# primus-labs/primus-fhe

Hardware: AMD Instinct MI355X
Metric: NTT/sec at N=2^16, 3-prime RNS (forward limb-NTTs, batch 4096 RNS polynomials per GPU) (higher is better)
Workload: dtype u64; 1 GPU; BASELINE configs[2] shape: N=2^16, 3-prime RNS (61-bit), batch=4096 per GPU, forward DCRT NTT in place (config 3'); log_n=16, batch_per_gpu=4096

## Files before the change

primus-fhe_amd/csrc/pfhe_ntt.hip:

```cpp
#include <algorithm>
#include <cstdio>
#include <cstdlib>
#include <vector>

#include "pfhe_common.hpp"
#include "pfhe_modmath.hpp"
#include "pfhe_ntt_device.hpp"

namespace pfhe {

template <bool INV>
__global__ void ntt_tiny_kernel(u64 *__restrict__ data, const NttPrime *__restrict__ primes, u32 L, u32 log_n,
                                u64 npolys, u32 lazy) {
    u64 pid = (u64)blockIdx.x * blockDim.x + threadIdx.x;
    if (pid >= npolys) return;
    const ShoupArith ar(primes + pid % L);
    const u32 n = 1u << log_n;
    u64 *x = data + pid * n;
    if (!INV) {
        for (u32 p = log_n; p-- > 0;) {
            for (u32 e = 0; e < n; ++e) {
                if (e & (1u << p)) continue;
                fwd_bfly(ar, x[e], x[e | (1u << p)], ar.fwd_tw((n + e) >> (p + 1)));
            }
// ... 72 lines not shown
}
template <class A, int K, int VEC, bool INV, bool FINAL>
__global__ __launch_bounds__(256) void ntt_strided_oop_kernel(u64 *__restrict__ dst, const u64 *__restrict__ src,
                                                              const NttPrime *__restrict__ primes, u32 L, u32 log_n, u32 log_s,
                                                              u64 total_threads, u32 lazy) {
    strided_pass_body<A, K, VEC, INV, FINAL, false>(dst, src, primes, L, log_n, log_s,
                                                    (u64)blockIdx.x * blockDim.x + threadIdx.x, total_threads, lazy);
}


struct NoHook {
    __device__ __forceinline__ void operator()() const {}
};
template <class A, int LOGB, bool INV, bool MUL, int LOGE = 4, class Hook = NoHook, bool NTIO = false, class Hook2 = NoHook>
__device__ __forceinline__ void block_pass_body(u64 *__restrict__ data, const u64 *src, const NttPrime *__restrict__ primes, u32 L,
                                                u32 log_n, u64 total_blocks, u32 lazy, const u64 *__restrict__ mul,
                                                u64 mul_polys, u64 *__restrict__ lds_raw, u64 first_block,
                                                Hook after_stage = Hook(), Hook2 before_store = Hook2()) {
    using Cfg = BlockCfg<LOGB, LOGE>;
    constexpr bool kNt = !std::is_same<Hook, NoHook>::value || NTIO;
    constexpr int NV = Cfg::E / 2;
    constexpr bool kWL = wave_local_vectors<LOGB, LOGE>() && !(INV && A::kMont && !std::is_same<Hook, NoHook>::value);
    const u32 tid = threadIdx.x;
    const u32 sub = Cfg::BPW == 1 ? 0u : tid / Cfg::TPB;
    const u32 lt = Cfg::BPW == 1 ? tid : tid % Cfg::TPB;
    u64 blk = first_block * Cfg::BPW + sub;
    const bool valid = blk < total_blocks;
    if (!valid) blk = 0;
    const u32 log_nb = log_n - LOGB;
    const u64 pid = blk >> log_nb;
    const u32 bi = (u32)(blk & ((1ull << log_nb) - 1));
    const u32 limb = (u32)(pid % L);
    const A ar(primes + limb);
    const u32 n = 1u << log_n;
    const u32 eblk = bi << LOGB;
    u64 *__restrict__ gptr = data + pid * n + eblk;
    const u64 *sgptr = src + pid * n + eblk;
    u64 *__restrict__ lds = lds_raw + (size_t)sub * Cfg::LDS_WORDS;

    constexpr bool kDirectLoad = !INV && !MUL && Cfg::BPW == 1 && (LOGB - LOGE) >= 6 &&
                                 !std::is_same<Hook, NoHook>::value && !A::kPacked
        ;
    u64x2 io[NV];
    u64 x[Cfg::E];
    if constexpr (kDirectLoad) {
#pragma unroll
        for (int k = 0; k < Cfg::E; ++k)
#ifdef PFHE_NOMEM
            x[k] = (u64)lt * 0x9E3779B97F4A7C15ull + (u64)k + lazy;
#else
            x[k] = valid ? __builtin_nontemporal_load(sgptr + ((u32)k << (LOGB - LOGE)) + lt) : 0ull;
#endif
        after_stage();
        block_forward_core<A, LOGB, false, LOGE>(ar, x, lds, n, eblk, lt, lazy != 0);
        lds_put_layout<0, LOGE>(x, lds, lt);
        sync_vectors_layout0<LOGB, LOGE, kWL>();
        lds_get_vectors<LOGB, LOGE, kWL>(io, lds, lt);
        before_store();
#ifdef PFHE_NOMEM
        if (lazy == 0xdeadu)
#endif
        if (valid) store_block_vectors<LOGB, LOGE, kNt, kWL>(io, gptr, lt);
        return;
    }
    if (valid) {
        load_block_vectors<LOGB, LOGE, kNt, kWL>(io, sgptr, lt);
    } else {
#pragma unroll
        for (int j = 0; j < NV; ++j) io[j] = u64x2{0, 0};
    }
    if constexpr (MUL) {
        u64x2 mv[NV];
        if (valid) {
            const u64 mpoly = mul_polys == (u64)L ? (u64)limb : pid;
            load_block_vectors<LOGB, LOGE, kNt, kWL>(mv, mul + mpoly * n + eblk, lt);
        } else {
#pragma unroll
            for (int j = 0; j < NV; ++j) mv[j] = u64x2{0, 0};
        }
#pragma unroll
        for (int j = 0; j < NV; ++j) {
            io[j].x = ar.mul_any(io[j].x, mv[j].x);
            io[j].y = ar.mul_any(io[j].y, mv[j].y);
        }
    }
    lds_put_vectors<LOGB, LOGE, kWL>(io, lds, lt);
    if constexpr (INV) sync_vectors_layout0<LOGB, LOGE, kWL>();
    else __syncthreads();
    if constexpr (!INV) after_stage();
    if constexpr (!INV) {
        lds_get_layout<LOGB - LOGE, LOGE>(x, lds, lt);
        block_forward_core<A, LOGB, false, LOGE>(ar, x, lds, n, eblk, lt, lazy != 0);
        lds_put_layout<0, LOGE>(x, lds, lt);
    } else {
        lds_get_layout<0, LOGE>(x, lds, lt);
        block_inverse_core<A, LOGB, false, LOGE, Hook>(ar, x, lds, n, eblk, lt, log_n == LOGB, lazy != 0, after_stage);
        constexpr bool kDirectStore = Cfg::BPW == 1 && (LOGB - LOGE) >= 6 && !A::kPacked
            ;
        if constexpr (kDirectStore) {
            before_store();
            if (valid) {
#pragma unroll
                for (int k = 0; k < Cfg::E; ++k)
                    gstore<(kNt && (std::is_same<Hook, NoHook>::value || kPipeIntermediateNt))>(
                        gptr + ((u32)k << (LOGB - LOGE)) + lt, x[k]);
            }
            return;
// ... 144 lines not shown

template <class A, int LOGB, bool INV, bool MUL>
__device__ __forceinline__ void ntt_pipe_body(
    u64 *__restrict__ blk_data, u64 blk_total, u64 *__restrict__ str_data, u64 str_total,
    const NttPrime *__restrict__ primes, u32 L, u32 lazy, const u64 *__restrict__ mul, u64 mul_polys) {
    constexpr int K = 4, TPB = BlockCfg<LOGB>::TPB;
    static_assert(BlockCfg<LOGB>::BPW == 1 && (1 << LOGB) / TPB == (1 << K), "16 blocks and 16 chunks per polynomial");
    constexpr u32 log_n = LOGB + K, n = 1u << log_n;
    extern __shared__ __attribute__((aligned(16))) u64 lds_raw[];
    const u64 chunk = blockIdx.x;
    const bool has_str = chunk < str_total;
    u64 *__restrict__ sp = str_data + (chunk >> 4) * n + (chunk & 15) * TPB + threadIdx.x;
    u64 sx[1 << K][1];
    const auto issue = [&]() {
        if (has_str) {
#pragma unroll
#ifdef PFHE_NOMEM
            for (int k = 0; k < (1 << K); ++k) sx[k][0] = (u64)threadIdx.x * 0xBF58476D1CE4E5B9ull + (u64)k + lazy;
#else
            for (int k = 0; k < (1 << K); ++k) sx[k][0] = __builtin_nontemporal_load(sp + ((u64)k << LOGB));
#endif
        }
    };
    const auto landed = [&]() {
        if (!INV && has_str) {
#pragma unroll
            for (int k = 0; k < (1 << K); ++k) asm volatile("" : "+v"(sx[k][0]));
        }
    };
    if (chunk < blk_total) {
        block_pass_body<A, LOGB, INV, MUL, 4, decltype(issue), false, decltype(landed)>(
            blk_data, blk_data, primes, L, log_n, blk_total, INV ? 0u : lazy, mul, mul_polys, lds_raw, chunk, issue, landed);
    } else {
        issue();
        landed();
    }
    if (has_str) {
        const A ar(primes + (chunk >> 4) % L);
        if constexpr (!INV) strided_forward_regs<A, K, 1, true>(ar, sx, n, 0u, LOGB);
        else strided_inverse_regs<A, K, 1, true>(ar, sx, n, 0u, LOGB, lazy != 0);
#ifdef PFHE_NOMEM
        if (lazy == 0xdeadu)
#endif
#pragma unroll
        for (int k = 0; k < (1 << K); ++k) gstore<(INV || kPipeIntermediateNt)>(sp + ((u64)k << LOGB), sx[k][0]);
    }
}

template <class A, int LOGB>
__global__ __launch_bounds__(BlockCfg<LOGB>::THREADS) __attribute__((amdgpu_waves_per_eu(4, 4))) void ntt_pipe_fwd_kernel(
    u64 *__restrict__ blk_data, u64 blk_total, u64 *__restrict__ str_data, u64 str_total,
    const NttPrime *__restrict__ primes, u32 L, u32 lazy) {
    ntt_pipe_body<A, LOGB, false, false>(blk_data, blk_total, str_data, str_total, primes, L, lazy, nullptr, 0);
}
template <class A, int LOGB, bool MUL>
__global__ __launch_bounds__(BlockCfg<LOGB>::THREADS) __attribute__((amdgpu_waves_per_eu(4, 4))) void ntt_pipe_inv_kernel(
    u64 *__restrict__ blk_data, u64 blk_total, u64 *__restrict__ str_data, u64 str_total,
    const NttPrime *__restrict__ primes, u32 L, u32 lazy, const u64 *__restrict__ mul, u64 mul_polys) {
    ntt_pipe_body<A, LOGB, true, MUL>(blk_data, blk_total, str_data, str_total, primes, L, lazy, mul, mul_polys);
}

template <class A, int LOGB, class HookA = NoHook, class HookM = NoHook, class HookL = NoLateHook, bool NT = false, bool MNT = false>
__device__ __forceinline__ void block_mid_body(const A &ar, u64 *__restrict__ gptr, const u64 *__restrict__ mptr, bool valid,
                                               u32 n, u32 eblk, bool final_block, u64 *__restrict__ lds,
                                               HookA after_load = HookA(), HookM mid = HookM(), HookL late = HookL()) {
    using Cfg = BlockCfg<LOGB>;
    static_assert(Cfg::BPW == 1 && LOGB - 4 >= 6, "one block per workgroup, whole waves per register layout");
    constexpr int NV = Cfg::E / 2, POS0 = LOGB - 4;
    u64 x[Cfg::E];
    {
        const u32 lt = opaque_tid();
#pragma unroll
        for (int k = 0; k < Cfg::E; ++k) x[k] = valid ? __builtin_nontemporal_load(gptr + ((u32)k << POS0) + lt) : 0ull;
        after_load();
        block_forward_core<A, LOGB, false, 4, NoLateHook, true>(ar, x, lds, n, eblk, lt, true);
        lds_put_layout<0>(x, lds, lt);
    }
    {
        const u32 lt = opaque_tid();
        u64x2 io[NV], mv[NV];
        if (valid) {
            load_block_vectors<LOGB, 4, MNT>(mv, mptr, lt);
        } else {
#pragma unroll
            for (int j = 0; j < NV; ++j) mv[j] = u64x2{0, 0};
        }
        sync_vectors_layout0<LOGB>();
        lds_get_vectors<LOGB>(io, lds, lt);
#pragma unroll
        for (int j = 0; j < NV; ++j) {
            io[j].x = ar.mul_any(io[j].x, mv[j].x);
            io[j].y = ar.mul_any(io[j].y, mv[j].y);
        }
        lds_put_vectors<LOGB>(io, lds, lt);
    }
    mid();
    sync_vectors_layout0<LOGB>();
    {
        const u32 lt = opaque_tid();
        lds_get_layout<0>(x, lds, lt);
        block_inverse_core<A, LOGB, false, 4, HookL>(ar, x, lds, n, eblk, lt, final_block, false, late);
    }
    if (valid) {
        const u32 lt = opaque_tid();
#pragma unroll
        for (int k = 0; k < Cfg::E; ++k) gstore<NT>(gptr + ((u32)k << POS0) + lt, x[k]);
// ... 306 lines not shown
        }
        return dispatch_strided<A, false, false>(k, data, primes, L, log_n, log_s, npolys, false, s);
    }
    if (i == 0) return dispatch_strided<A, true, true>(k, data, primes, L, log_n, log_s, npolys, lazy, s);
    return dispatch_strided<A, true, false>(k, data, primes, L, log_n, log_s, npolys, false, s);
}

int pass_dev(const NttPlan &plan, bool persistent, const NttPrime *primes, u32 L, u32 log_n, int arith, u64 *data, u64 npolys,
             bool inverse, int index, bool lazy, hipStream_t s, const u64 *mul, u64 mul_polys) {
    if (index < 0 || index >= plan.passes()) return PFHE_ERR_BAD_ARGUMENT;
    if (plan.tiny) {
        if (arith == kArithB32 || mul) return PFHE_ERR_UNSUPPORTED;
        return launch_tiny(inverse, primes, L, log_n, data, npolys, lazy, s);
    }
    if (persistent)
        return with_arith(arith, [&](auto a) {
            using A = typename decltype(a)::type;
            return inverse ? launch_persist<A, true>(data, primes, L, npolys, lazy, s)
                           : launch_persist<A, false>(data, primes, L, npolys, lazy, s);
        });
    return with_arith<true>(arith, [&](auto a) {
        return run_pass<typename decltype(a)::type>(plan, primes, L, log_n, data, npolys, inverse, index, lazy, s, mul, mul_polys);
    });
}

void pass_name(const NttPlan &plan, bool inverse, int index, char *buf, size_t cap) {
    if (plan.tiny) {
        std::snprintf(buf, cap, "ntt_tiny_kernel");
        return;
    }
    const int block_at = inverse ? 0 : plan.n_strided;
    if (index == block_at) {
        std::snprintf(buf, cap, "ntt_block_kernel<%d,%s>", plan.block_log, inverse ? "inv" : "fwd");
    } else {
        const int i = inverse ? plan.n_strided - index : index;
        std::snprintf(buf, cap, "ntt_strided_kernel<K=%d,%s>", plan.strided[i], inverse ? "inv" : "fwd");
    }
}

}

static int env_int(const char *name, int lo, int hi) {
    const char *e = std::getenv(name);
    if (!e) return 0;
    const int v = std::atoi(e);
    return v >= lo && v <= hi ? v : 0;
}

NttTuning NttTuning::from_env() {
    NttTuning t;
    t.pipe_tiles = env_int("PFHE_PIPE_TILES", 2, 4096);
    t.pipelined = std::getenv("PFHE_DISABLE_PIPELINED") == nullptr;
    t.pipelined_min_mb = env_int("PFHE_PIPELINED_MIN_MB", 1, 1 << 20);
    return t;
}

NttPlan make_ntt_plan(u32 log_n, int arith) {
    NttPlan p;
    if (log_n <= 3) {
        p.tiny = true;
        return p;
    }
    if (log_n <= kMaxSinglePassLog) {
        p.block_log = (int)log_n;
        return p;
    }
    p.block_log = kTwoPassBlockLog;
    if (arith == kArithB32 && log_n == 15) p.block_log = 11;
    int rest = (int)log_n - p.block_log;
    int passes = (rest + 4) / 5;
    for (int i = 0; i < passes; ++i) {
        int k = (rest + (passes - i) - 1) / (passes - i);
        p.strided[p.n_strided++] = k;
        rest -= k;
    }
    return p;
}

int ntt_num_passes(u32 log_n, int arith) { return make_ntt_plan(log_n, arith).passes(); }

void ntt_pass_name(u32 log_n, bool inverse, int index, char *buf, size_t cap, int arith) {
    pass_name(make_ntt_plan(log_n, arith), inverse, index, buf, cap);
}

int ntt_pass_dev(const NttPrime *primes, u32 L, u32 log_n, int arith, u64 *data, u64 npolys, bool inverse, int index,
                 bool lazy, hipStream_t s, const u64 *mul, u64 mul_polys) {
    const NttPlan plan = make_ntt_plan(log_n, arith);
    return pass_dev(plan, mul == nullptr && takes_persistent(plan, arith, npolys), primes, L, log_n, arith, data, npolys,
                    inverse, index, lazy, s, mul, mul_polys);
}

namespace {
constexpr u64 kPipelinedMinBytes = 256ull << 20;
constexpr u64 kPipelinedTileBytes = 256ull << 20;
constexpr int kPipelinedMaxTiles = 64;

int pipelined_tiles(const NttPlan &plan, u32 L, u32 log_n, int arith, u64 npolys, bool inverse, bool has_mul,
                    const NttTuning &tune) {
    const u64 bytes = (npolys << log_n) * sizeof(u64);
    const bool b32 = arith == kArithB32;
    const bool shape = log_n == (b32 ? 15u : 16u) && plan.n_strided == 1 && plan.block_log == (b32 ? 11 : 12);
    if (!(tune.pipelined && shape && (!has_mul || inverse) && npolys % L == 0 &&
          bytes >= (tune.pipelined_min_mb ? (u64)tune.pipelined_min_mb << 20
                                           : b32 ? 4 * kPipelinedMinBytes : kPipelinedMinBytes)))
        return 0;
    const u64 tile_bytes = b32 ? 2 * kPipelinedTileBytes : kPipelinedTileBytes;
    int pt = tune.pipe_tiles ? tune.pipe_tiles
                                : (int)std::min<u64>((bytes + tile_bytes / 2) / tile_bytes, (u64)kPipelinedMaxTiles);
    if (pt < 2) pt = 2;
    if (pt > kPipelinedMaxTiles) pt = kPipelinedMaxTiles;
    if ((u64)pt > npolys / L) pt = (int)(npolys / L);
    return pt;
}

enum class NttOp { kTransform, kInverseMul, kPolymul };
struct NttForm {
    enum Kind { kPasses, kPersistent, kPipelined } kind = kPasses;
    int tiles = 0;
};
NttForm ntt_form(const NttPlan &plan, u32 L, u32 log_n, int arith, u64 npolys, bool inverse, NttOp op, const NttTuning &tune) {
    NttForm f;
    f.tiles = pipelined_tiles(plan, L, log_n, arith, npolys, inverse, op != NttOp::kTransform, tune);
    if (f.tiles >= 1) f.kind = NttForm::kPipelined;
    else if (op != NttOp::kInverseMul && takes_persistent(plan, arith, npolys)) f.kind = NttForm::kPersistent;
    return f;
}

struct PipeTiles {
    u64 *data;
    u64 npolys;
    const u64 *mul;
    u64 mul_polys;
    u32 L, log_n;
    int block_log, tiles;
    struct Tile {
        u64 *ptr = nullptr;
        u64 blocks = 0;
        const u64 *mul = nullptr;
        u64 mul_polys = 0;
    };
    Tile operator[](int k) const {
        Tile t;
        if (k < 0 || k >= tiles) return t;
        const u64 units = npolys / L, u0 = units * (u64)k / (u64)tiles, u1 = units * (u64)(k + 1) / (u64)tiles;
        t.ptr = data + ((u0 * L) << log_n);
        t.blocks = ((u1 - u0) * L) << (log_n - (u32)block_log);
        if (mul) {
            const bool each = mul_polys == npolys;
            t.mul = each ? mul + ((u0 * L) << log_n) : mul;
            t.mul_polys = each ? (u1 - u0) * L : mul_polys;
        }
        return t;
    }
};
}

template <class A, int LOGB>
static int transform_pipelined(const NttPrime *primes, u32 L, u64 *data, u64 npolys, bool inverse, bool lazy,
                               hipStream_t s, int tiles, const u64 *mul, u64 mul_polys) {
    constexpr size_t lds_bytes = (size_t)BlockCfg<LOGB>::LDS_WORDS * sizeof(u64);
    constexpr u32 threads = BlockCfg<LOGB>::THREADS;
    const PipeTiles split{data, npolys, mul, mul_polys, L, LOGB + 4, LOGB, tiles};
    for (int k = 0; k <= tiles; ++k) {
        const PipeTiles::Tile b = split[inverse ? k : k - 1], st = split[inverse ? k - 1 : k];
        const u64 grid = std::max(b.blocks, st.blocks);
        if constexpr (!A::kPacked) {
            if (inverse && mul) {
                PFHE_TRY((launch<ntt_pipe_inv_kernel<A, LOGB, true>>(grid, threads, lds_bytes, s, b.ptr, b.blocks, st.ptr, st.blocks,
                                                                     primes, L, lazy ? 1u : 0u, b.mul, b.mul_polys)));
                continue;
            }
        }
        if (inverse)
            PFHE_TRY((launch<ntt_pipe_inv_kernel<A, LOGB, false>>(grid, threads, lds_bytes, s, b.ptr, b.blocks, st.ptr, st.blocks,
                                                                  primes, L, lazy ? 1u : 0u, b.mul, b.mul_polys)));
        else
            PFHE_TRY((launch<ntt_pipe_fwd_kernel<A, LOGB>>(grid, threads, lds_bytes, s, b.ptr, b.blocks, st.ptr, st.blocks, primes,
                                                           L, lazy ? 1u : 0u)));
    }
    return PFHE_OK;
}

int ntt_transform_form(u32 L, u32 log_n, int arith, u64 npolys, bool inverse, const NttTuning &tune, char *buf, size_t cap) {
    const NttPlan plan = make_ntt_plan(log_n, arith);
    const NttForm form = ntt_form(plan, L, log_n, arith, npolys, inverse, NttOp::kTransform, tune);
    if (form.kind == NttForm::kPipelined) {
        std::snprintf(buf, cap, inverse ? "ntt_pipe_inv_kernel" : "ntt_pipe_fwd_kernel");
        return form.tiles + 1;
    }
    if (form.kind == NttForm::kPersistent) {
        std::snprintf(buf, cap, "ntt_persist_kernel<14,%s>", inverse ? "inv" : "fwd");
        return 1;
    }
    size_t at = 0;
    buf[0] = 0;
    for (int i = 0; i < plan.passes() && at + 1 < cap; ++i) {
        char one[96];
        pass_name(plan, inverse, i, one, sizeof one);
        at += (size_t)std::snprintf(buf + at, cap - at, "%s%s", i ? " + " : "", one);
    }
    return plan.passes();
}

static int transform(const NttPrime *primes, u32 L, u32 log_n, int arith, u64 *data, u64 npolys, bool inverse,
                     bool lazy, hipStream_t s, const NttTuning &tune, const u64 *mul = nullptr, u64 mul_polys = 0) {
    const NttPlan plan = make_ntt_plan(log_n, arith);
    const NttForm form = ntt_form(plan, L, log_n, arith, npolys, inverse, mul ? NttOp::kInverseMul : NttOp::kTransform, tune);
    if (form.kind == NttForm::kPipelined)
        return with_arith<true>(arith, [&](auto a) {
            using A = typename decltype(a)::type;
            return transform_pipelined<A, A::kPacked ? 11 : 12>(primes, L, data, npolys, inverse, lazy, s, form.tiles, mul, mul_polys);
        });
    for (int i = 0; i < plan.passes(); ++i)
        PFHE_TRY(pass_dev(plan, form.kind == NttForm::kPersistent, primes, L, log_n, arith, data, npolys, inverse, i, lazy, s,
                          i == 0 ? mul : nullptr, mul_polys));
    return PFHE_OK;
}

int ntt_forward_dev(const NttPrime *primes, u32 L, u32 log_n, int arith, u64 *data, u64 npolys, bool lazy,
                    hipStream_t s, const NttTuning &tune) {
    return transform(primes, L, log_n, arith, data, npolys, false, lazy, s, tune);
}

int ntt_inverse_dev(const NttPrime *primes, u32 L, u32 log_n, int arith, u64 *data, u64 npolys, bool lazy,
                    hipStream_t s, const NttTuning &tune) {
    return transform(primes, L, log_n, arith, data, npolys, true, lazy, s, tune);
}

template <class A>
static int through_dev_two_pass(const NttPlan &plan, const NttPrime *primes, u32 L, u32 log_n, u64 *io, u64 *scratch, u64 npolys,
                                bool inverse, bool lazy, hipStream_t s) {
    const int k = plan.strided[0];
    const u32 log_s = log_n - k;
    const u64 sthreads = (npolys << (log_n - k)) >> (k == 5 ? 0 : 1), sgrid = (sthreads + 255) / 256;
    const u64 blocks = npolys << (log_n - 12);
    if (sgrid > kMaxGrid || blocks > kMaxGrid) return PFHE_ERR_UNSUPPORTED;
    constexpr size_t lds_bytes = (size_t)BlockCfg<12>::LDS_WORDS * sizeof(u64);
    const auto strided = [&](auto kc, u64 *dst, const u64 *src) {
        constexpr int K = decltype(kc)::value, VEC = K == 5 ? 1 : 2;
        if (!inverse)
            hipLaunchKernelGGL((ntt_strided_oop_kernel<A, K, VEC, false, false>), dim3((u32)sgrid), dim3(256), 0, s, dst, src, primes,
                               L, log_n, log_s, sthreads, 0u);
        else
            hipLaunchKernelGGL((ntt_strided_oop_kernel<A, K, VEC, true, true>), dim3((u32)sgrid), dim3(256), 0, s, dst, src, primes,
                               L, log_n, log_s, sthreads, lazy ? 1u : 0u);
    };
    const auto strided_k = [&](u64 *dst, const u64 *src) {
        if (k == 3) strided(std::integral_constant<int, 3>{}, dst, src);
        else if (k == 4) strided(std::integral_constant<int, 4>{}, dst, src);
        else strided(std::integral_constant<int, 5>{}, dst, src);
    };
    if (!inverse) {
        strided_k(scratch, io);
        hipLaunchKernelGGL((ntt_block_oop_kernel<A, false>), dim3((u32)blocks), dim3(BlockCfg<12>::THREADS), lds_bytes, s, io,
                           scratch, primes, L, log_n, blocks, lazy ? 1u : 0u);
    } else {
        hipLaunchKernelGGL((ntt_block_oop_kernel<A, true>), dim3((u32)blocks), dim3(BlockCfg<12>::THREADS), lds_bytes, s, scratch,
                           io, primes, L, log_n, blocks, 0u);
        strided_k(io, scratch);
    }
    PFHE_HIP(hipGetLastError());
    return PFHE_OK;
}

// ... 145 lines not shown
```

primus-fhe_amd/csrc/pfhe_ntt_device.hpp:

```cpp
#pragma once

#include <type_traits>

#include "pfhe_common.hpp"
#include "pfhe_modmath.hpp"
#if defined(__HIPCC__)
#include "pfhe_mont_asm.hpp"
#include "pfhe_pm_asm.hpp"
#endif

namespace pfhe {

constexpr u32 kMaxSinglePassLog = 14;
constexpr int kTwoPassBlockLog = 12;

struct NttPlan {
    bool tiny = false;
    int n_strided = 0;
    int strided[4] = {0, 0, 0, 0};
    int block_log = 0;
    int passes() const { return tiny ? 1 : n_strided + 1; }
};

struct NttTuning {
    int pipe_tiles = 0;
    bool pipelined = true;
    int pipelined_min_mb = 0;
    static NttTuning from_env();
};
NttPlan make_ntt_plan(u32 log_n, int arith = 0);

enum : int { kArithShoup = 0, kArithPm = 1, kArithB32 = 2, kArithMont = 3 };
int ntt_forward_dev(const NttPrime *primes, u32 L, u32 log_n, int arith, u64 *data, u64 npolys, bool lazy,
                    hipStream_t s, const NttTuning &tune = NttTuning());
int ntt_transform_form(u32 L, u32 log_n, int arith, u64 npolys, bool inverse, const NttTuning &tune, char *buf, size_t cap);
int ntt_inverse_dev(const NttPrime *primes, u32 L, u32 log_n, int arith, u64 *data, u64 npolys, bool lazy,
                    hipStream_t s, const NttTuning &tune = NttTuning());
int ntt_transform_through_dev(const NttPrime *primes, u32 L, u32 log_n, int arith, u64 *io, u64 *scratch, u64 npolys,
                              bool inverse, bool lazy, hipStream_t s, const NttTuning &tune = NttTuning());
int ntt_inverse_mul_dev(const NttPrime *primes, u32 L, u32 log_n, int arith, u64 *data, u64 npolys, const u64 *mul,
                        u64 mul_polys, hipStream_t s, const NttTuning &tune = NttTuning());
int ntt_polymul_dev(const NttPrime *primes, u32 L, u32 log_n, int arith, u64 *data, u64 npolys, const u64 *mul,
                    u64 mul_polys, hipStream_t s, const NttTuning &tune = NttTuning());
int ntt32_transform_dev(const NttPrime *primes, u32 L, u32 log_n, u32 *data, u64 npolys, bool inverse, bool lazy,
                        hipStream_t s, const NttTuning &tune = NttTuning());

int ntt_num_passes(u32 log_n, int arith = 0);
void ntt_pass_name(u32 log_n, bool inverse, int index, char *buf, size_t cap, int arith = 0);
int ntt_pass_dev(const NttPrime *primes, u32 L, u32 log_n, int arith, u64 *data, u64 npolys, bool inverse,
                 int index, bool lazy, hipStream_t s, const u64 *mul = nullptr, u64 mul_polys = 0);

constexpr u64 kMaxGrid = 0x7fffffffull;
int launch_grid(u64 count, u32 *grid);

#if defined(__HIPCC__)

struct ShoupArith;
struct PmArith;
struct MontArith;
struct B32Arith;
template <class A>
struct ArithTag {
    using type = A;
};
template <bool B32 = false, class F>
inline int with_arith(int arith, F &&f) {
    if constexpr (B32) {
        if (arith == kArithB32) return f(ArithTag<B32Arith>{});
    }
    if (arith == kArithMont) return f(ArithTag<MontArith>{});
    return arith == kArithPm ? f(ArithTag<PmArith>{}) : f(ArithTag<ShoupArith>{});
}

#if defined(__HIP_DEVICE_COMPILE__) && defined(__AMDGCN_WAVEFRONT_SIZE) && __AMDGCN_WAVEFRONT_SIZE != 64
#error "libpfhe_hip is written for wave64 targets (gfx950)"
#endif

typedef u64 u64x2 __attribute__((ext_vector_type(2)));
typedef const u64x2 __attribute__((address_space(1))) *GCVec2Ptr;
typedef u64x2 __attribute__((address_space(1))) *GVec2Ptr;
// ... 494 lines not shown
            }
        }
    }
    if constexpr (FINAL) {
#pragma unroll
        for (int v = 0; v < R / 2; ++v)
#pragma unroll
            for (int c = 0; c < VEC; ++c) inv_final_bfly(ar, x[v][c], x[v + R / 2][c], lazy);
    }
}

template <int LOGB, int LOGE = 4>
struct BlockCfg {
    static_assert(LOGB >= 4 && LOGB <= 14, "block pass handles 2^4 .. 2^14 coefficients");
    static_assert(LOGE == 3 || LOGE == 4, "8 or 16 coefficients per thread");
    static constexpr int B = 1 << LOGB;
    static constexpr int E = 1 << LOGE;
    static constexpr int TPB = B >> LOGE;
    static_assert(TPB <= 1024, "a block must fit one workgroup");
    static constexpr int kMinWg = 64;
    static constexpr int THREADS = TPB > kMinWg ? TPB : kMinWg;
    static constexpr int BPW = THREADS / TPB;
    static constexpr int LDS_WORDS = B + B / 8;
};

__device__ __forceinline__ u32 lds_phi(u32 e) { return e + ((e >> 4) << 1); }

template <int POS, int LOGE = 4>
__device__ __forceinline__ u32 layout(u32 lt, int k) {
    if constexpr (POS == 0) {
        return (lt << LOGE) | (u32)k;
    } else {
        return ((lt >> POS) << (POS + LOGE)) | ((u32)k << POS) | (lt & ((1u << POS) - 1));
    }
}

template <int POS, bool UNIFORM>
__device__ __forceinline__ u32 maybe_uniform(u32 v) {
    if constexpr (UNIFORM && POS >= 6) {
        return __builtin_amdgcn_readfirstlane(v);
    } else {
        return v;
    }
}

template <int LOGE>
__device__ __forceinline__ u32 last_table_off(u32 n, u32 e0, int j, int u) {
    constexpr int S = 4 - LOGE;
    const u32 g = e0 >> LOGE, h = g & ((1u << S) - 1), g16 = g >> S;
    const u32 uu = (h << (LOGE - 1 - j)) + (u32)u;
    return (((8u >> j) - 1) + uu) * (n >> 4) + g16;
}

template <class A, int POS, int JHI, int JLO, bool UNIFORM, int LOGE = 4, bool EVEN = false>
__device__ __forceinline__ void fwd_regpass(const A &ar, u64 (&x)[1 << LOGE], u32 n_plus_e, u32 n) {
    constexpr int E = 1 << LOGE;
#ifdef PFHE_SKELETON
#pragma unroll
    for (int v = 0; v < E / 2; ++v) {
        x[v] += x[v | (E / 2)];
        x[v | (E / 2)] ^= x[v];
    }
    return;
#endif
#pragma unroll
    for (int j = JHI; j >= JLO; --j) {
        const u32 base = maybe_uniform<POS, UNIFORM>(n_plus_e >> (POS + j + 1));
        constexpr bool kUni = UNIFORM && POS >= 6;
        typename A::Tw w[E / 2];
        const auto load_tw = [&](int u) {
            if constexpr (POS == 0 && A::kLastTables) w[u] = ar.fwd_tw_last(last_table_off<LOGE>(n, n_plus_e - n, j, u));
            else w[u] = ar.fwd_tw(base + u);
        };
        const int ntw = E >> (j + 1);
        if constexpr (A::kWide || A::kMont) {
            const int group = (kUni || ntw <= 4) ? ntw : 4;
#pragma unroll
            for (int u0 = 0; u0 < ntw; u0 += group) {
#pragma unroll
                for (int u = u0; u < u0 + group; ++u) load_tw(u);
#pragma unroll
                for (int b = u0 << j; b < ((u0 + group) << j); b += 2) {
                    const int ua = b >> j, va = b & ((1 << j) - 1), ub = (b + 1) >> j, vb = (b + 1) & ((1 << j) - 1);
                    const int a0 = (ua << (j + 1)) | va, a1 = a0 | (1 << j), b0 = (ub << (j + 1)) | vb, b1 = b0 | (1 << j);
                    if constexpr (A::kMont) mont_fwd_bfly2<kUni>(ar, x[a0], x[a1], w[ua], x[b0], x[b1], w[ub]);
                    else if ((((POS + j) & 1) != 0) != EVEN) pm_fwd_bfly2<true, kUni>(ar, x[a0], x[a1], w[ua], x[b0], x[b1], w[ub]);
                    else pm_fwd_bfly2<false, kUni>(ar, x[a0], x[a1], w[ua], x[b0], x[b1], w[ub]);
                }
            }
            continue;
        }
#pragma unroll
        for (int u = 0; u < ntw; ++u) load_tw(u);
#pragma unroll
        for (int u = 0; u < ntw; ++u) {
#pragma unroll
            for (int v = 0; v < (1 << j); ++v) {
                const int k0 = (u << (j + 1)) | v, k1 = k0 | (1 << j);
                if ((((POS + j) & 1) != 0) != EVEN) fwd_bfly<true, kUni>(ar, x[k0], x[k1], w[u]);
                else fwd_bfly<false, kUni>(ar, x[k0], x[k1], w[u]);
            }
        }
    }
}

template <class A, int POS, int JLO, int JHI, bool UNIFORM, int LOGE = 4>
__device__ __forceinline__ void inv_regpass(const A &ar, u64 (&x)[1 << LOGE], u32 n, u32 e_abs, bool final_stage,
                                            bool lazy) {
    constexpr int E = 1 << LOGE;
#pragma unroll
    for (int j = JLO; j <= JHI; ++j) {
        const u32 p = POS + j;
        if (j == JHI && final_stage) {
#pragma unroll
            for (int v = 0; v < E / 2; ++v) inv_final_bfly(ar, x[v], x[v | (E / 2)], lazy);
        } else {
            const u32 base = maybe_uniform<POS, UNIFORM>(1 + n - (n >> p) + (e_abs >> (p + 1)));
            constexpr bool kUni = UNIFORM && POS >= 6;
            typename A::Tw w[E / 2];
            const int ntw = E >> (j + 1);
#pragma unroll
            for (int u = 0; u < ntw; ++u) {
                if constexpr (POS == 0 && A::kLastTables) w[u] = ar.inv_tw_last(last_table_off<LOGE>(n, e_abs, j, u));
                else w[u] = ar.inv_tw(base + u);
            }
            if constexpr (A::kWide || A::kMont) {
#pragma unroll
                for (int b = 0; b < E / 2; b += 2) {
                    const int ua = b >> j, va = b & ((1 << j) - 1), ub = (b + 1) >> j, vb = (b + 1) & ((1 << j) - 1);
                    const int a0 = (ua << (j + 1)) | va, a1 = a0 | (1 << j), b0 = (ub << (j + 1)) | vb, b1 = b0 | (1 << j);
                    if constexpr (A::kMont) mont_inv_bfly2<kUni>(ar, x[a0], x[a1], w[ua], x[b0], x[b1], w[ub]);
                    else pm_inv_bfly2<kUni>(ar, x[a0], x[a1], w[ua], x[b0], x[b1], w[ub]);
                }
                continue;
            }
#pragma unroll
            for (int u = 0; u < ntw; ++u) {
#pragma unroll
                for (int v = 0; v < (1 << j); ++v) {
                    const int k0 = (u << (j + 1)) | v, k1 = k0 | (1 << j);
                    inv_bfly<kUni>(ar, x[k0], x[k1], w[u]);
                }
            }
        }
    }
}

template <int POS>
__host__ __device__ constexpr u32 lds_koff(int k) {
    return ((u32)k << POS) + 2u * (((u32)k << POS) >> 4);
}

template <int POS, int LOGE = 4>
__device__ __forceinline__ void lds_get_layout(u64 (&x)[1 << LOGE], const u64 *__restrict__ lds, u32 lt) {
    const u64 *__restrict__ base = lds + lds_phi(layout<POS, LOGE>(lt, 0));
#pragma unroll
    for (int k = 0; k < (1 << LOGE); ++k) x[k] = base[lds_koff<POS>(k)];
}

template <int POS, int LOGE = 4>
__device__ __forceinline__ void lds_put_layout(const u64 (&x)[1 << LOGE], u64 *__restrict__ lds, u32 lt) {
    u64 *__restrict__ base = lds + lds_phi(layout<POS, LOGE>(lt, 0));
#pragma unroll
    for (int k = 0; k < (1 << LOGE); ++k) base[lds_koff<POS>(k)] = x[k];
}

template <int FROM, int TO, bool FIRST, int LOGE = 4>
__device__ __forceinline__ void lds_exchange(u64 (&x)[1 << LOGE], u64 *__restrict__ lds, u32 lt) {
    constexpr bool kLead = FIRST, kWaveLocal = (FROM > TO ? FROM : TO) <= 6;
    if constexpr (kLead) __syncthreads();
    lds_put_layout<FROM, LOGE>(x, lds, lt);
    if constexpr (kWaveLocal) {
        __builtin_amdgcn_fence(__ATOMIC_RELEASE, "wavefront");
        __builtin_amdgcn_wave_barrier();
        __builtin_amdgcn_fence(__ATOMIC_ACQUIRE, "wavefront");
    } else {
        __syncthreads();
    }
    lds_get_layout<TO, LOGE>(x, lds, lt);
}

constexpr bool kPipeIntermediateNt = false;

struct NoLateHook {
    __device__ __forceinline__ void operator()() const {}
};
template <class A, int LOGB, int POS, bool FIRST = false, int LOGE = 4, class Late = NoLateHook, bool EVEN = false>
__device__ __forceinline__ void fwd_chain(const A &ar, u64 (&x)[1 << LOGE], u64 *__restrict__ lds, u32 n, u32 eblk, u32 lt,
                                          Late before_last = Late()) {
    constexpr bool UNI = BlockCfg<LOGB, LOGE>::TPB >= 64;
    if constexpr (POS > 0) {
        constexpr int NPOS = POS >= LOGE ? POS - LOGE : 0;
        constexpr int JHI = POS >= LOGE ? LOGE - 1 : POS - 1;
        asm volatile("" : "+v"(lt));
        lds_exchange<POS, NPOS, FIRST, LOGE>(x, lds, lt);
        if constexpr (NPOS == 0) before_last();
        fwd_regpass<A, NPOS, JHI, 0, UNI, LOGE, EVEN>(ar, x, n + eblk + layout<NPOS, LOGE>(lt, 0), n);
        fwd_chain<A, LOGB, NPOS, false, LOGE, Late, EVEN>(ar, x, lds, n, eblk, lt, before_last);
    }
}

template <class A, int LOGB, bool LEAD = true, int LOGE = 4, class Late = NoLateHook, bool RAW = false>
__device__ __forceinline__ void block_forward_core(const A &ar, u64 (&x)[1 << LOGE], u64 *__restrict__ lds, u32 n,
                                                   u32 eblk, u32 lt, bool lazy, Late before_last = Late()) {
    constexpr int POS0 = LOGB - LOGE, E = 1 << LOGE;
    constexpr bool UNI = BlockCfg<LOGB, LOGE>::TPB >= 64;
    constexpr bool EVEN = RAW && A::kWide;
    fwd_regpass<A, POS0, LOGE - 1, 0, UNI, LOGE, EVEN>(ar, x, n + eblk + layout<POS0, LOGE>(lt, 0), n);
    fwd_chain<A, LOGB, POS0, LEAD, LOGE, Late, EVEN>(ar, x, lds, n, eblk, lt, before_last);
    if constexpr (RAW && (A::kWide || A::kMont)) return;
    if constexpr (A::kPacked) {
        if constexpr (LOGE == 4) {
            const u32 off0 = 15u * (n >> 4) + (eblk >> 4) + lt;
#pragma unroll
            for (int k = 0; k < E; ++k) x[k] = ar.fwd_intra_tw(x[k], ar.fwd_tw_last(off0 + (u32)k * (n >> 4)));
        } else {
#pragma unroll
            for (int k = 0; k < E; ++k) x[k] = ar.fwd_intra(x[k], n + eblk + layout<0, LOGE>(lt, k));
        }
    }
    if constexpr (A::kWide) {
        if (!lazy) {
#pragma unroll
            for (int k = 0; k < E; k += 2) pm_canon2(ar, x[k], x[k + 1]);
        } else
        {
#pragma unroll
            for (int k = 0; k < E; ++k) x[k] = fwd_finish(ar, x[k], lazy);
        }
    } else if constexpr (A::kMont) {
        ar.canon_regs(x);
    } else if (!lazy) {
#pragma unroll
        for (int k = 0; k < E; ++k) x[k] = ar.reduce_4q(x[k]);
    }
}

template <class A, int LOGB, int POS, bool FIRST = false, int LOGE = 4, class Late = NoLateHook, int HOOK_AT = 0>
__device__ __forceinline__ void inv_chain(const A &ar, u64 (&x)[1 << LOGE], u64 *__restrict__ lds, u32 n, u32 eblk, u32 lt,
                                          bool final_block, bool lazy, Late before_last = Late()) {
    constexpr bool UNI = BlockCfg<LOGB, LOGE>::TPB >= 64;
    constexpr int DONE = POS + LOGE;
    if constexpr (DONE < LOGB) {
        constexpr int NPOS = DONE <= LOGB - LOGE ? DONE : LOGB - LOGE;
        constexpr int JLO = DONE - NPOS;
        constexpr bool LAST = NPOS + LOGE >= LOGB;
        asm volatile("" : "+v"(lt));
        lds_exchange<POS, NPOS, FIRST, LOGE>(x, lds, lt);
        constexpr int AFTER = (LOGB - NPOS - LOGE + LOGE - 1) / LOGE;
        if constexpr (AFTER == HOOK_AT) before_last();
        inv_regpass<A, NPOS, JLO, LOGE - 1, UNI, LOGE>(ar, x, n, eblk + layout<NPOS, LOGE>(lt, 0), LAST && final_block, lazy);
        inv_chain<A, LOGB, NPOS, false, LOGE, Late, HOOK_AT>(ar, x, lds, n, eblk, lt, final_block, lazy, before_last);
    }
}

template <class A, int LOGB, bool LEAD = true, int LOGE = 4, class Late = NoLateHook, int HOOK_AT = 0>
__device__ __forceinline__ void block_inverse_core(const A &ar, u64 (&x)[1 << LOGE], u64 *__restrict__ lds, u32 n,
                                                   u32 eblk, u32 lt, bool final_block, bool lazy, Late before_last = Late()) {
    constexpr bool UNI = BlockCfg<LOGB, LOGE>::TPB >= 64;
    if constexpr (A::kPacked) {
        if constexpr (LOGE == 4) {
            const u32 off0 = 15u * (n >> 4) + (eblk >> 4) + lt;
// ... 108 lines not shown
```

Before: 2.658 million NTT/s.

## Add 8-coefficient forward pipelined NTT kernel with permlane32 swap and tight twiddle scheduling

Adds a new forward pipelined kernel that uses 8 coefficients per thread (LOGE=3) with twice the threads and waves_per_eu of 6 instead of 4, aiming at higher occupancy and better latency hiding. The strided tail pass is split across two lanes per column, which exchange halves through permlane32_swap so the last butterfly stage and the stores stay in registers. A 'tight' regpass variant loads twiddles in small groups and uses asm dependencies to keep register pressure down. The new kernel is on by default for PM arithmetic on forward transforms. It adds register-layout complexity and extra cross-lane traffic.

```diff
diff --git a/primus-fhe_amd/csrc/pfhe_ntt.hip b/primus-fhe_amd/csrc/pfhe_ntt.hip
--- a/primus-fhe_amd/csrc/pfhe_ntt.hip
+++ b/primus-fhe_amd/csrc/pfhe_ntt.hip
@@ -148,7 +148,7 @@
             x[k] = valid ? __builtin_nontemporal_load(sgptr + ((u32)k << (LOGB - LOGE)) + lt) : 0ull;
 #endif
         after_stage();
-        block_forward_core<A, LOGB, false, LOGE>(ar, x, lds, n, eblk, lt, lazy != 0);
+        block_forward_core<A, LOGB, false, LOGE, NoLateHook, false, LOGE == 3>(ar, x, lds, n, eblk, lt, lazy != 0);
         lds_put_layout<0, LOGE>(x, lds, lt);
         sync_vectors_layout0<LOGB, LOGE, kWL>();
         lds_get_vectors<LOGB, LOGE, kWL>(io, lds, lt);
@@ -399,6 +399,76 @@
     u64 *__restrict__ blk_data, u64 blk_total, u64 *__restrict__ str_data, u64 str_total,
     const NttPrime *__restrict__ primes, u32 L, u32 lazy) {
     ntt_pipe_body<A, LOGB, false, false>(blk_data, blk_total, str_data, str_total, primes, L, lazy, nullptr, 0);
+}
+__device__ __forceinline__ void permlane32_swap64(u64 &lo_keeps, u64 &hi_keeps) {
+    const auto a = __builtin_amdgcn_permlane32_swap((u32)lo_keeps, (u32)hi_keeps, false, false);
+    const auto b = __builtin_amdgcn_permlane32_swap((u32)(lo_keeps >> 32), (u32)(hi_keeps >> 32), false, false);
+    lo_keeps = ((u64)b[0] << 32) | a[0];
+    hi_keeps = ((u64)b[1] << 32) | a[1];
+}
+template <class A, int LOGB>
+__global__ __launch_bounds__((BlockCfg<LOGB, 3>::THREADS)) __attribute__((amdgpu_waves_per_eu(6, 6))) void ntt_pipe_fwd8_kernel(
+    u64 *__restrict__ blk_data, u64 blk_total, u64 *__restrict__ str_data, u64 str_total,
+    const NttPrime *__restrict__ primes, u32 L, u32 lazy) {
+    constexpr int K = 4, R = 1 << (K - 1), COLS = 1 << (LOGB - K);
+    static_assert(BlockCfg<LOGB, 3>::BPW == 1 && BlockCfg<LOGB, 3>::THREADS == 2 * COLS, "two lanes per column of the chunk");
+    constexpr u32 log_n = LOGB + K, n = 1u << log_n;
+    extern __shared__ __attribute__((aligned(16))) u64 lds_raw[];
+    const u64 chunk = blockIdx.x;
+    const bool has_str = chunk < str_total;
+    u64 *__restrict__ const cbase = str_data + (chunk >> 4) * n + (chunk & 15) * COLS;
+    const auto column = [](u32 t) { return ((t >> 6) << 5) | (t & 31u); };
+    const auto half = [](u32 t) { return (t >> 5) & 1u; };
+    u64 sx[R];
+    const auto issue = [&]() {
+        if (has_str) {
+            const u32 t = opaque_tid();
+            const u64 *__restrict__ sp = cbase + column(t) + ((u64)half(t) << LOGB);
+#pragma unroll
+            for (int r = 0; r < R; ++r) sx[r] = __builtin_nontemporal_load(sp + ((u64)r << (LOGB + 1)));
+        }
+    };
+    const auto landed = [&]() {
+        if (has_str) {
+#pragma unroll
+            for (int r = 0; r < R; ++r) asm volatile("" : "+v"(sx[r]));
+        }
+    };
+    if (chunk < blk_total) {
+        block_pass_body<A, LOGB, false, false, 3, decltype(issue), false, decltype(landed)>(
+            blk_data, blk_data, primes, L, log_n, blk_total, lazy, nullptr, 0, lds_raw, chunk, issue, landed);
+    } else {
+        issue();
+        landed();
+    }
+    if (has_str) {
+        const A ar(primes + (chunk >> 4) % L);
+#pragma unroll
+        for (int j = K - 2; j >= 0; --j) {
+            const u32 base = n >> (LOGB + j + 2);
+#pragma unroll
+            for (int u = 0; u < (R >> (j + 1)); ++u) {
+                const typename A::Tw w = ar.fwd_tw(base + u);
+#pragma unroll
+                for (int v = 0; v < (1 << j); ++v) {
+                    const int k0 = (u << (j + 1)) | v, k1 = k0 | (1 << j);
+                    if (j & 1) fwd_bfly<true, true>(ar, sx[k0], sx[k1], w);
+                    else fwd_bfly<false, true>(ar, sx[k0], sx[k1], w);
+                }
+            }
+        }
+#pragma unroll
+        for (int i = 0; i < R / 2; ++i) permlane32_swap64(sx[i], sx[R / 2 + i]);
+        const u32 t = opaque_tid();
+        const u32 tw0 = (n >> (LOGB + 1)) + half(t) * (R / 2);
+        u64 *__restrict__ sp = cbase + column(t) + ((u64)(half(t) * R) << LOGB);
+#pragma unroll
+        for (int i = 0; i < R / 2; ++i) {
+            fwd_bfly<true, false>(ar, sx[i], sx[R / 2 + i], ar.fwd_tw(tw0 + i));
+            gstore<kPipeIntermediateNt>(sp + ((u64)(2 * i) << LOGB), sx[i]);
+            gstore<kPipeIntermediateNt>(sp + ((u64)(2 * i + 1) << LOGB), sx[R / 2 + i]);
+        }
+    }
 }
 template <class A, int LOGB, bool MUL>
 __global__ __launch_bounds__(BlockCfg<LOGB>::THREADS) __attribute__((amdgpu_waves_per_eu(4, 4))) void ntt_pipe_inv_kernel(
@@ -811,6 +881,8 @@
     t.pipe_tiles = env_int("PFHE_PIPE_TILES", 2, 4096);
     t.pipelined = std::getenv("PFHE_DISABLE_PIPELINED") == nullptr;
     t.pipelined_min_mb = env_int("PFHE_PIPELINED_MIN_MB", 1, 1 << 20);
+    const char *fwd8 = std::getenv("PFHE_PIPE_FWD8");
+    t.pipe_fwd8 = !(fwd8 && fwd8[0] == '0' && fwd8[1] == 0);
     return t;
 }
 
@@ -876,11 +948,15 @@
 struct NttForm {
     enum Kind { kPasses, kPersistent, kPipelined } kind = kPasses;
     int tiles = 0;
+    bool fwd8 = false;
 };
 NttForm ntt_form(const NttPlan &plan, u32 L, u32 log_n, int arith, u64 npolys, bool inverse, NttOp op, const NttTuning &tune) {
     NttForm f;
     f.tiles = pipelined_tiles(plan, L, log_n, arith, npolys, inverse, op != NttOp::kTransform, tune);
-    if (f.tiles >= 1) f.kind = NttForm::kPipelined;
+    if (f.tiles >= 1) {
+        f.kind = NttForm::kPipelined;
+        f.fwd8 = tune.pipe_fwd8 && arith == kArithPm && !inverse && op == NttOp::kTransform;
+    }
     else if (op != NttOp::kInverseMul && takes_persistent(plan, arith, npolys)) f.kind = NttForm::kPersistent;
     return f;
 }
@@ -916,7 +992,7 @@
 
 template <class A, int LOGB>
 static int transform_pipelined(const NttPrime *primes, u32 L, u64 *data, u64 npolys, bool inverse, bool lazy,
-                               hipStream_t s, int tiles, const u64 *mul, u64 mul_polys) {
+                               hipStream_t s, int tiles, bool fwd8, const u64 *mul, u64 mul_polys) {
     constexpr size_t lds_bytes = (size_t)BlockCfg<LOGB>::LDS_WORDS * sizeof(u64);
     constexpr u32 threads = BlockCfg<LOGB>::THREADS;
     const PipeTiles split{data, npolys, mul, mul_polys, L, LOGB + 4, LOGB, tiles};
@@ -930,6 +1006,13 @@
                 continue;
             }
         }
+        if constexpr (std::is_same<A, PmArith>::value) {
+            if (!inverse && fwd8) {
+                PFHE_TRY((launch<ntt_pipe_fwd8_kernel<A, LOGB>>(grid, BlockCfg<LOGB, 3>::THREADS, lds_bytes, s, b.ptr, b.blocks, st.ptr,
+                                                                st.blocks, primes, L, lazy ? 1u : 0u)));
+                continue;
+            }
+        }
         if (inverse)
             PFHE_TRY((launch<ntt_pipe_inv_kernel<A, LOGB, false>>(grid, threads, lds_bytes, s, b.ptr, b.blocks, st.ptr, st.blocks,
                                                                   primes, L, lazy ? 1u : 0u, b.mul, b.mul_polys)));
@@ -968,7 +1051,8 @@
     if (form.kind == NttForm::kPipelined)
         return with_arith<true>(arith, [&](auto a) {
             using A = typename decltype(a)::type;
-            return transform_pipelined<A, A::kPacked ? 11 : 12>(primes, L, data, npolys, inverse, lazy, s, form.tiles, mul, mul_polys);
+            return transform_pipelined<A, A::kPacked ? 11 : 12>(primes, L, data, npolys, inverse, lazy, s, form.tiles, form.fwd8, mul,
+                                                                mul_polys);
         });
     for (int i = 0; i < plan.passes(); ++i)
         PFHE_TRY(pass_dev(plan, form.kind == NttForm::kPersistent, primes, L, log_n, arith, data, npolys, inverse, i, lazy, s,
diff --git a/primus-fhe_amd/csrc/pfhe_ntt_device.hpp b/primus-fhe_amd/csrc/pfhe_ntt_device.hpp
--- a/primus-fhe_amd/csrc/pfhe_ntt_device.hpp
+++ b/primus-fhe_amd/csrc/pfhe_ntt_device.hpp
@@ -26,6 +26,7 @@
     int pipe_tiles = 0;
     bool pipelined = true;
     int pipelined_min_mb = 0;
+    bool pipe_fwd8 = true;
     static NttTuning from_env();
 };
 NttPlan make_ntt_plan(u32 log_n, int arith = 0);
@@ -626,9 +627,12 @@
     return (((8u >> j) - 1) + uu) * (n >> 4) + g16;
 }
 
-template <class A, int POS, int JHI, int JLO, bool UNIFORM, int LOGE = 4, bool EVEN = false>
+template <class A, int POS, int JHI, int JLO, bool UNIFORM, int LOGE = 4, bool EVEN = false, bool TIGHT = false>
 __device__ __forceinline__ void fwd_regpass(const A &ar, u64 (&x)[1 << LOGE], u32 n_plus_e, u32 n) {
     constexpr int E = 1 << LOGE;
+    static_assert(!TIGHT || LOGE == 3, "the tight form is written for 8 coefficients per thread");
+    u32 npe[2] = {n_plus_e, n_plus_e};
+    int gi = 0;
 #ifdef PFHE_SKELETON
 #pragma unroll
     for (int v = 0; v < E / 2; ++v) {
@@ -641,14 +645,19 @@
     for (int j = JHI; j >= JLO; --j) {
         const u32 base = maybe_uniform<POS, UNIFORM>(n_plus_e >> (POS + j + 1));
         constexpr bool kUni = UNIFORM && POS >= 6;
+        constexpr bool kTight = TIGHT && !kUni && (A::kWide || A::kMont);
         typename A::Tw w[E / 2];
         const auto load_tw = [&](int u) {
-            if constexpr (POS == 0 && A::kLastTables) w[u] = ar.fwd_tw_last(last_table_off<LOGE>(n, n_plus_e - n, j, u));
+            if constexpr (kTight) {
+                const u32 e = npe[0];
+                if constexpr (POS == 0 && A::kLastTables) w[u] = ar.fwd_tw_last(last_table_off<LOGE>(n, e - n, j, u));
+                else w[u] = ar.fwd_tw((e >> (POS + j + 1)) + u);
+            } else if constexpr (POS == 0 && A::kLastTables) w[u] = ar.fwd_tw_last(last_table_off<LOGE>(n, n_plus_e - n, j, u));
             else w[u] = ar.fwd_tw(base + u);
         };
         const int ntw = E >> (j + 1);
         if constexpr (A::kWide || A::kMont) {
-            const int group = (kUni || ntw <= 4) ? ntw : 4;
+            const int group = kTight ? (ntw < 2 ? ntw : 2) : (kUni || ntw <= 4) ? ntw : 4;
 #pragma unroll
             for (int u0 = 0; u0 < ntw; u0 += group) {
 #pragma unroll
@@ -660,6 +669,12 @@
                     if constexpr (A::kMont) mont_fwd_bfly2<kUni>(ar, x[a0], x[a1], w[ua], x[b0], x[b1], w[ub]);
                     else if ((((POS + j) & 1) != 0) != EVEN) pm_fwd_bfly2<true, kUni>(ar, x[a0], x[a1], w[ua], x[b0], x[b1], w[ub]);
                     else pm_fwd_bfly2<false, kUni>(ar, x[a0], x[a1], w[ua], x[b0], x[b1], w[ub]);
+                }
+                if constexpr (kTight) {
+                    u32 e = n_plus_e;
+                    asm("" : "+v"(e) : "v"(x[0]), "v"(x[1]), "v"(x[2]), "v"(x[3]), "v"(x[4]), "v"(x[5]), "v"(x[6]), "v"(x[7]));
+                    npe[0] = e;
+                    ++gi;
                 }
             }
             continue;
@@ -759,7 +774,7 @@
 struct NoLateHook {
     __device__ __forceinline__ void operator()() const {}
 };
-template <class A, int LOGB, int POS, bool FIRST = false, int LOGE = 4, class Late = NoLateHook, bool EVEN = false>
+template <class A, int LOGB, int POS, bool FIRST = false, int LOGE = 4, class Late = NoLateHook, bool EVEN = false, bool TIGHT = false>
 __device__ __forceinline__ void fwd_chain(const A &ar, u64 (&x)[1 << LOGE], u64 *__restrict__ lds, u32 n, u32 eblk, u32 lt,
                                           Late before_last = Late()) {
     constexpr bool UNI = BlockCfg<LOGB, LOGE>::TPB >= 64;
@@ -769,19 +784,19 @@
         asm volatile("" : "+v"(lt));
         lds_exchange<POS, NPOS, FIRST, LOGE>(x, lds, lt);
         if constexpr (NPOS == 0) before_last();
-        fwd_regpass<A, NPOS, JHI, 0, UNI, LOGE, EVEN>(ar, x, n + eblk + layout<NPOS, LOGE>(lt, 0), n);
-        fwd_chain<A, LOGB, NPOS, false, LOGE, Late, EVEN>(ar, x, lds, n, eblk, lt, before_last);
-    }
-}
-
-template <class A, int LOGB, bool LEAD = true, int LOGE = 4, class Late = NoLateHook, bool RAW = false>
+        fwd_regpass<A, NPOS, JHI, 0, UNI, LOGE, EVEN, TIGHT>(ar, x, n + eblk + layout<NPOS, LOGE>(lt, 0), n);
+        fwd_chain<A, LOGB, NPOS, false, LOGE, Late, EVEN, TIGHT>(ar, x, lds, n, eblk, lt, before_last);
+    }
+}
+
+template <class A, int LOGB, bool LEAD = true, int LOGE = 4, class Late = NoLateHook, bool RAW = false, bool TIGHT = false>
 __device__ __forceinline__ void block_forward_core(const A &ar, u64 (&x)[1 << LOGE], u64 *__restrict__ lds, u32 n,
                                                    u32 eblk, u32 lt, bool lazy, Late before_last = Late()) {
     constexpr int POS0 = LOGB - LOGE, E = 1 << LOGE;
     constexpr bool UNI = BlockCfg<LOGB, LOGE>::TPB >= 64;
     constexpr bool EVEN = RAW && A::kWide;
-    fwd_regpass<A, POS0, LOGE - 1, 0, UNI, LOGE, EVEN>(ar, x, n + eblk + layout<POS0, LOGE>(lt, 0), n);
-    fwd_chain<A, LOGB, POS0, LEAD, LOGE, Late, EVEN>(ar, x, lds, n, eblk, lt, before_last);
+    fwd_regpass<A, POS0, LOGE - 1, 0, UNI, LOGE, EVEN, TIGHT>(ar, x, n + eblk + layout<POS0, LOGE>(lt, 0), n);
+    fwd_chain<A, LOGB, POS0, LEAD, LOGE, Late, EVEN, TIGHT>(ar, x, lds, n, eblk, lt, before_last);
     if constexpr (RAW && (A::kWide || A::kMont)) return;
     if constexpr (A::kPacked) {
         if constexpr (LOGE == 4) {
```

Measured after the change: 2.565 million NTT/s. -3.5%, worse.
